# retinal-information-processing-lab/gaussian_processes

Measured on AMD Instinct MI355X. Metric: GP fits/sec (kernel+chol+solve+grad loglik) at N=8192 d=256, higher is better.
Workload: dtype f64; 1 GPU; N=8192 d=256 single cell f64, one M-step closure evaluation with 6 gradients (BASELINE configs[2], headline); N=8192, d=256, parallelism=independent units over 1 GPU(s), one process per GPU, no data-path collective

## Files before the change

gaussian_processes_amd/_lib.py:

```python
from __future__ import annotations

import ctypes
import os

from .build import lib_path

vp, i32, i64, f64 = ctypes.c_void_p, ctypes.c_int, ctypes.c_int64, ctypes.c_double
pd = ctypes.POINTER(ctypes.c_double)

_SIGS = {
    "gpfit_version": (i32, []),
    "gpfit_last_error": (ctypes.c_char_p, []),
    "gpfit_dgemm": (i32, [vp, i32, i32, i32, i32, i32, f64, vp, i64, vp, i64, f64, vp, i64, i32, i32, i32]),
    "gpfit_dgemm_ex": (i32, [vp, i32, i32, i32, i32, i32, f64, vp, i64, vp, i64, f64, vp, i64, i32, i32, i32, i32, i32]),
    "gpfit_ctx_create": (i32, [i32, i64, i64, i64, ctypes.POINTER(vp)]),
    "gpfit_ctx_destroy": (None, [vp]),
    "gpfit_check_limits": (i32, [pd, pd, pd]),
    "gpfit_localker_mask": (i32, [pd, i32, i32, vp, ctypes.POINTER(i64)]),
    "gpfit_localker": (i32, [vp, vp, pd, i32, i32, vp, i64, vp, vp]),
    "gpfit_acosker": (i32, [vp, vp, f64, vp, i64, i64, vp, i64, i64, i64, vp, i64, vp, vp, i64, vp]),
    "gpfit_acosker_pullback": (i32, [vp, vp, f64, vp, i64, i64, vp, i64, i64, i64, vp, i64, vp, i64, vp, vp, i64, pd]),
    "gpfit_acosker_diag": (i32, [vp, vp, f64, vp, i64, i64, i64, vp, i64, vp, vp, vp]),
    "gpfit_fit_eval": (i32, [vp, vp, pd, pd, pd, i32, i32, vp, i64, i64, vp, vp, vp, i64, f64, f64, i32, pd,
                             vp, vp, vp]),
    "gpfit_potrf": (i32, [vp, vp, vp, i64, i64, vp, i64, vp, i64, pd, ctypes.POINTER(i32)]),
    "gpfit_potrf_append": (i32, [vp, vp, vp, i64, vp, i64, i64, vp, pd, ctypes.POINTER(i32)]),
    "gpfit_estep": (i32, [vp, vp, vp, i64, i64, vp, vp, vp, f64, vp, vp, i64]),
    "gpfit_estep_projected": (i32, [vp, vp, vp, i64, vp, i64, vp, i64, i64, i64, vp, vp, vp, f64, vp, vp, i64, vp, vp,
                                    vp]),
# ... 65 lines not shown
```

gaussian_processes_amd/csrc/api_core.hip:

```cpp
#include "common.h"
#include "gpfit_mi355x.h"

namespace gpfit {
static thread_local std::string g_err;
void set_error(const std::string& m) { g_err = m; }
}

extern "C" {

int gpfit_version(void) { return GPFIT_VERSION; }

const char* gpfit_last_error(void) { return gpfit::g_err.c_str(); }

int gpfit_dgemm_ex(void* stream, int a_kmajor, int b_kmajor, int M, int N, int K, double alpha,
                   const double* A, int64_t lda, const double* B, int64_t ldb, double beta, double* C,
                   int64_t ldc, int out_lower, int a_tri, int b_tri, int walk, int tile);

int gpfit_dgemm(void* stream, int a_kmajor, int b_kmajor, int M, int N, int K, double alpha,
                const double* A, int64_t lda, const double* B, int64_t ldb, double beta, double* C,
                int64_t ldc, int out_lower, int a_tri, int b_tri) {
  return gpfit_dgemm_ex(stream, a_kmajor, b_kmajor, M, N, K, alpha, A, lda, B, ldb, beta, C, ldc, out_lower,
                        a_tri, b_tri, 0, 0);
}

int gpfit_dgemm_ex(void* stream, int a_kmajor, int b_kmajor, int M, int N, int K, double alpha,
                   const double* A, int64_t lda, const double* B, int64_t ldb, double beta, double* C,
                   int64_t ldc, int out_lower, int a_tri, int b_tri, int walk, int tile) {
  if ((M & 1) || (N & 1)) {
    gpfit::set_error("gpfit_dgemm: M and N must be even");
    return -3;
  }
  gpfit::GemmArgs g{};
  g.A = A; g.B = B; g.C = C;
  g.lda = lda; g.ldb = ldb; g.ldc = ldc;
  g.M = M; g.N = N; g.K = K;
  g.alpha = alpha; g.beta = beta;
  g.a_kmajor = a_kmajor; g.b_kmajor = b_kmajor;
  g.out_lower = out_lower; g.a_tri = a_tri; g.b_tri = b_tri;
  g.batch = 1; g.split_k = 1; g.reverse = walk & 15; g.tile = tile;
  g.half_occ = (walk >> 4) & 1;
  return gpfit::launch_gemm(g, (hipStream_t)stream);
}

}
```

gaussian_processes_amd/csrc/common.h:

```cpp
#pragma once
#include <hip/hip_runtime.h>
#include <stdint.h>
#include <stdio.h>
#include <string>

namespace gpfit {

constexpr double PI32 = 3.1415927410125732;

constexpr int TILE = 128;
constexpr int TRMV_ROWS = 128;
constexpr int KTILE = 16;

void set_error(const std::string& msg);

#define GP_HIP(expr)                                                                     \
  do {                                                                                   \
    hipError_t _e = (expr);                                                              \
    if (_e != hipSuccess) {                                                              \
      gpfit::set_error(std::string(#expr) + ": " + hipGetErrorString(_e));               \
      return -100;                                                                       \
    }                                                                                    \
  } while (0)

// ... 8 lines not shown
  R* C;
  int64_t lda, ldb, ldc;
  int M, N, K;
  double alpha, beta;
  int a_kmajor, b_kmajor;
  int out_lower;
  int a_tri, b_tri;
  int batch;
  int64_t sA, sB, sC;
  int split_k;
  int tile;
  int reverse;
  int workspace;
  void* sk_ws;
  int tile_limit;
  int half_occ;
  const int* sched;
  int sched_blocks;
  int epi;
  R* aux;
  double* sumsq;
  int nptr;
  const R* Ap[GEMM_MAXB];
  const R* Bp[GEMM_MAXB];
  R* Cp[GEMM_MAXB];
  R* auxp[GEMM_MAXB];
  double* sumsqp[GEMM_MAXB];
};
using GemmArgs = GemmArgsT<double>;

constexpr size_t SK_WS_BYTES = (size_t)2 * 512 * TILE * TILE * sizeof(double);

template <typename R> constexpr int ktile_of() { return 128 / (int)sizeof(R); }

template <typename R> int launch_gemm(const GemmArgsT<R>& a, hipStream_t s);
template <typename R> int gemm_pick_tile(const GemmArgsT<R>& a);
template <typename R> int launch_gemm_streamk(const GemmArgsT<R>& a, hipStream_t s);
template <typename R> int launch_gemm_plain(const GemmArgsT<R>& a, hipStream_t s);
template <typename R> bool gemm_pair_ok(const GemmArgsT<R>& a, const GemmArgsT<R>& b);
template <typename R> int launch_gemm_pair(const GemmArgsT<R>& a, const GemmArgsT<R>& b, hipStream_t s);
template <typename R> int launch_gemm_xcd(const GemmArgsT<R>& a, hipStream_t s);
template <typename R> bool gemm_epilogue_ok(const GemmArgsT<R>& a);
template <typename R> bool gemm_streamk_applies(const GemmArgsT<R>& a);
template <typename R> bool gemm_streamk_carries(const GemmArgsT<R>& a);
template <typename R> int gemm_sumsq_entries(const GemmArgsT<R>& a);
template <typename R> bool gemm_xcd_applies(const GemmArgsT<R>& a);

template <typename R>
// ... 20 lines not shown
```

gaussian_processes_amd/csrc/fit.hip:

```cpp
#include "context.h"
#include "gpfit_mi355x.h"

#include <algorithm>
#include <chrono>
#include <cmath>
#include <cstdlib>
#include <cstring>
#include <limits>

namespace gpfit {

static thread_local gpfit_ctx* g_prof = nullptr;
static thread_local void* g_main_sk_ws = nullptr;

static const int* walks() {
  static int w[7] = {3, 2, 1, 9, 9, 2, 2};
  static bool init = false;
  if (!init) {
    init = true;
    if (const char* e = getenv("GPFIT_WALKS")) {
      int v[7];
      if (sscanf(e, "%d,%d,%d,%d,%d,%d,%d", &v[0], &v[1], &v[2], &v[3], &v[4], &v[5], &v[6]) == 7)
        for (int i = 0; i < 7; ++i) w[i] = v[i];
    }
// ... 245 lines not shown
    bt.n = B.nb;
    for (int b = 0; b < B.nb; ++b) {
      bt.A[b] = B.A[b] + off(r0, r0); bt.L[b] = B.L[b] + off(r0, r0); bt.Li[b] = B.Li[b] + off(r0, r0);
      bt.info[b] = B.info[b];
    }
    bt.lda = bt.ldl = bt.ldi = ld;
    bt.info_base = r0;
    return launch_chol_leaf_batch(bt, s);
  }
  const int k = n / TILE;
  const int n1 = ((k + 1) / 2) * TILE, n2 = n - n1;
  const int r1 = r0 + n1;
  GP_TRY(potrf_lockstep<R>(B, r0, n1, all, s));
  GP_TRY(bgemm<R>(B, s, all, 0, 0, n2, n1, n1, 1.0, B.A, off(r1, r0), B.Li, off(r0, r0), 0.0, B.L, off(r1, r0), 0, 0, 2,
                  walks()[0], B.ws, B.sk_ws));
  hipEvent_t joined = nullptr;
  if (need && B.ctx && B.side_min > 0 && n >= B.side_min && B.ctx->side) {
    gpfit_ctx* c = B.ctx;
    auto next_event = [&]() {
      if (c->side_ev_next == (int)c->side_ev.size()) {
        hipEvent_t e = nullptr;
        (void)hipEventCreateWithFlags(&e, hipEventDisableTiming);
        c->side_ev.push_back(e);
      }
      return c->side_ev[c->side_ev_next++];
    };
    hipEvent_t fork = next_event();
    joined = next_event();
    GP_HIP(hipEventRecord(fork, s));
    GP_HIP(hipStreamWaitEvent(c->side, fork, 0));
    GP_TRY(bgemm<R>(B, c->side, need, 0, 1, n2, n1, n1, 1.0, B.L, off(r1, r0), B.Li, off(r0, r0), 0.0, B.Tmp, off(r1, r0), 0, 0,
                    1, walks()[1], 1, c->sk_ws[1]));
    GP_HIP(hipEventRecord(joined, c->side));
  }
  bool merged = false;
  if (need && !joined) {
    static const bool no_batch = getenv("GPFIT_NO_BATCH") != nullptr;
    const GemmArgsT<R> g2 = batch_args<R>(B, all, 0, 0, n2, n2, n1, -1.0, B.L, off(r1, r0), B.L, off(r1, r0), 1.0, B.A, off(r1, r1),
                                          1, 0, 0, 0);
    const GemmArgsT<R> g3 = batch_args<R>(B, need, 0, 1, n2, n1, n1, 1.0, B.L, off(r1, r0), B.Li, off(r0, r0), 0.0, B.Tmp,
                                          off(r1, r0), 0, 0, 1, walks()[1]);
    if (!no_batch && gemm_pair_ok(g2, g3)) {
      if (gemm_log_eval() >= 0 && g_eval_count == gemm_log_eval())
        fprintf(stderr, "[gpfit gemm] pair: M %d N %d K %d lower 1 nb %d + M %d N %d K %d btri 1 nb %d tile %d flops %.6e\n", g2.M, g2.N,
                g2.K, g2.nptr, g3.M, g3.N, g3.K, g3.nptr, gemm_pick_tile(g3), gemm_flops(g2) + gemm_flops(g3));
      ProfScope ps(s, g_prof ? gemm_flops(g2) + gemm_flops(g3) : 0.0, 3);
      GP_TRY(launch_gemm_pair(g2, g3, s));
      merged = true;
    }
  }
  if (!merged)
    GP_TRY(bgemm<R>(B, s, all, 0, 0, n2, n2, n1, -1.0, B.L, off(r1, r0), B.L, off(r1, r0), 1.0, B.A, off(r1, r1), 1, 0, 0, 0,
                    B.ws, B.sk_ws));
  GP_TRY(potrf_lockstep<R>(B, r1, n2, need | halves, s));
  if (need) {
    if (joined) GP_HIP(hipStreamWaitEvent(s, joined, 0));
    else if (!merged)
      GP_TRY(bgemm<R>(B, s, need, 0, 1, n2, n1, n1, 1.0, B.L, off(r1, r0), B.Li, off(r0, r0), 0.0, B.Tmp, off(r1, r0), 0, 0,
                      1, walks()[1], B.ws, B.sk_ws));
    GP_TRY(bgemm<R>(B, s, need, 0, 1, n2, n1, n2, -1.0, B.Li, off(r1, r1), B.Tmp, off(r1, r0), 0.0, B.Li, off(r1, r0), 0, 1, 0,
                    walks()[2], B.ws, B.sk_ws));
  }
  return 0;
}

template int potrf_lockstep<double>(const CholBatchT<double>&, int, int, uint32_t, hipStream_t, uint32_t);
template int potrf_lockstep<float>(const CholBatchT<float>&, int, int, uint32_t, hipStream_t, uint32_t);

// ... 289 lines not shown
  };
  c->phase_valid = false;
  phase(0, s);
  g_main_sk_ws = c->sk_ws[0];
  prof_begin(c);
  struct ProfGuard { gpfit_ctx* c; ~ProfGuard() { prof_end(c); } } prof_guard{c};
  GP_HIP(hipMemsetAsync(c->info, 0, 4 * sizeof(int), s));
  GP_HIP(hipMemcpyAsync(c->pix, c->pix_host, (size_t)d * sizeof(int), hipMemcpyHostToDevice, s));
  GP_HIP(hipMemsetAsync(RP(c->mpad), 0, (size_t)np * sizeof(R), s));
  GP_HIP(hipMemcpyAsync(RP(c->mpad), m, (size_t)n * sizeof(R), hipMemcpyDeviceToDevice, s));

  const bool reuse_V = (want_grad & 2) && c->lv_valid && c->lv_n == n && c->lv_bytes == (int)sizeof(R);
  const bool async_call = (want_grad & 4) != 0;
  const bool mixed_grad = (want_grad & 8) != 0 && sizeof(R) == 8 && (want_grad & 1);
  want_grad &= 1;
  static const int side_min_env = getenv("GPFIT_SIDE_MIN") ? atoi(getenv("GPFIT_SIDE_MIN")) : 1024;
  const int side_min = async_call ? 0 : side_min_env;
  if (!async_call) GP_TRY(ensure_side_stream(c));
  c->side_ev_next = 0;
  if (!reuse_V) {
    c->lv_valid = false; c->lv32_valid = false;
    GP_HIP(hipEventRecord(c->ev_fork, s));
    GP_HIP(hipStreamWaitEvent(c->aux, c->ev_fork, 0));
    GP_TRY(launch_pack_lower(V, ldv, n, RP(c->Vbuf), ld, np, c->aux));
    GP_HIP(hipEventRecord(c->ev_join, c->aux));
  }

  GP_TRY(launch_localker<R>(th, c->pix, d, dp, n_rows, n_cols, RP(c->Cmat), dp, nullptr, s));
  GP_TRY(launch_gather(X, ldx, n, c->pix, d, dp, np, RP(c->Xt), ld, RP(c->Xm), dp, s));
  GP_TRY(gemm<R>(s, 1, 1, dp, np, dp, 1.0, RP(c->Cmat), dp, RP(c->Xt), ld, 0.0, RP(c->XCt), ld, 0, 0, 0));
  GP_TRY(launch_qvec(RP(c->Xt), RP(c->XCt), ld, dp, n, np, s0sq, RP(c->Kvec), RP(c->q), s));
// ... 944 lines not shown
```

gaussian_processes_amd/csrc/gemm.hip:

```cpp
#include "gemm_core.h"

#include <algorithm>
#include <cstdlib>
#include <mutex>
#include <set>
#include <utility>

namespace gpfit {

template <typename R, bool A_KMAJOR, bool B_KMAJOR, bool EDGE, int T, int NS>
__device__ __forceinline__ bool gemm_tile_compute(const GemmArgsT<R>& p, int tiles_n, int ntiles, R* smem,
                                                  typename Real<R>::acc_t (&acc)[T / 32][T / 32], int& ti, int& tj,
                                                  int& row0, int& col0, R*& C) {
  constexpr int KT = Real<R>::KT;

  const int bid = (p.reverse & 1) ? (ntiles - 1 - (int)blockIdx.x) : (int)blockIdx.x;
  if (p.sched != nullptr) {
    const int e = p.sched[blockIdx.x];
    if (e < 0) return false;
    ti = e >> 16;
    tj = e & 0xffff;
  } else if (p.out_lower && (p.reverse & 2) && T == TILE) {
    const int nt = tiles_n;
    int j = (int)((2.0 * nt + 1.0 - sqrt((2.0 * nt + 1.0) * (2.0 * nt + 1.0) - 8.0 * (double)bid)) * 0.5);
    while (j > 0 && (long)j * nt - (long)j * (j - 1) / 2 > bid) --j;
    while ((long)(j + 1) * nt - (long)(j + 1) * j / 2 <= bid) ++j;
    tj = j;
    ti = j + (bid - (j * nt - j * (j - 1) / 2));
  } else if (p.out_lower) {
    lower_tile(bid, TILE / T, ti, tj);
  } else if (p.reverse & 2) {
    const int tiles_m = ntiles / tiles_n;
    tj = bid / tiles_m;
// ... 30 lines not shown
    kbeg = kbeg + s0 * KT;
    C += (int64_t)z * p.sC;
  }

#pragma unroll
  for (int i = 0; i < T / 32; ++i)
#pragma unroll
    for (int j = 0; j < T / 32; ++j) acc[i][j] = acc_zero<R>();

  gemm_mainloop<R, A_KMAJOR, B_KMAJOR, EDGE, T, 0, NS>(A, p.lda, B, p.ldb, p.M, p.N, row0, col0, kbeg, kend, smem, acc,
                                                       (p.reverse & 4) != 0);
  return true;
}

template <typename R, bool A_KMAJOR, bool B_KMAJOR, bool EDGE, int T, int NS, int EPI = 0>
__device__ __forceinline__ void gemm_tile_body(const GemmArgsT<R>& p, int tiles_n, int ntiles, R* smem) {
  typename Real<R>::acc_t acc[T / 32][T / 32];
  int ti, tj, row0, col0;
  R* C;
  if (!gemm_tile_compute<R, A_KMAJOR, B_KMAJOR, EDGE, T, NS>(p, tiles_n, ntiles, smem, acc, ti, tj, row0, col0, C)) return;

  const R alpha = (R)p.alpha, beta = (p.split_k > 1) ? (R)0 : (R)p.beta;
  const int64_t ldc = p.ldc;
  const int M = p.M, N = p.N;
  if constexpr (EPI != 0) {
    constexpr int epi = EPI;
    R* __restrict__ D = p.nptr > 0 ? p.auxp[blockIdx.y] : p.aux;
    double* __restrict__ sumsq = p.nptr > 0 ? p.sumsqp[blockIdx.y] : p.sumsq;
    double ss = 0.0;
    for_each_acc<R, T>(acc, row0, col0, [&](int row, int col, R v) {
      if (EDGE && !(row < M && col < N)) return;
      R o = alpha * v;
      R* c = C + (int64_t)row * ldc + col;
      if (epi & 4) {
        R* dd = D + (int64_t)row * ldc + col;
// ... 29 lines not shown
  } else {
    for_each_acc<R, T>(acc, row0, col0, [&](int row, int col, R v) {
      if (!EDGE || (row < M && col < N)) {
        R* c = C + (int64_t)row * ldc + col;
        *c = alpha * v + beta * (*c);
      }
    });
  }
}

template <typename R, bool A_KMAJOR, bool B_KMAJOR, bool EDGE, int T, int NS = 2>
__global__ __launch_bounds__(GEMM_THREADS, (T == 128 || NS > 2 ? 2 : 4)) void gemm_mfma_kernel(GemmArgsT<R> p,
                                                                                               int tiles_n,
                                                                                               int ntiles) {
  __shared__ __attribute__((aligned(16))) R smem[2 * NS * Real<R>::KT * T];
  gemm_tile_body<R, A_KMAJOR, B_KMAJOR, EDGE, T, NS>(p, tiles_n, ntiles, smem);
}

#ifdef GPFIT_CLOCK_STAMPS
__device__ long long g_gemm_clock[2][4096][2];
#endif

template <typename R, bool A_KMAJOR, bool B_KMAJOR>
__global__ __launch_bounds__(GEMM_THREADS, 2) void gemm_xcd_kernel(GemmArgsT<R> p, int tiles_n, int ntiles) {
  __shared__ __attribute__((aligned(16))) R smem[4 * Real<R>::KT * TILE];
#ifdef GPFIT_CLOCK_STAMPS
  const long long t0 = __builtin_amdgcn_s_memtime(), w0 = __builtin_amdgcn_s_memrealtime();
#endif
  gemm_tile_body<R, A_KMAJOR, B_KMAJOR, false, TILE, 2>(p, tiles_n, ntiles, smem);
#ifdef GPFIT_CLOCK_STAMPS
  if (threadIdx.x == 0 && blockIdx.x < 4096) {
    g_gemm_clock[B_KMAJOR ? 1 : 0][blockIdx.x][0] = (long long)__builtin_amdgcn_s_memtime() - t0;
    g_gemm_clock[B_KMAJOR ? 1 : 0][blockIdx.x][1] = (long long)__builtin_amdgcn_s_memrealtime() - w0;
  }
#endif
}

template <typename R, bool A_KMAJOR, bool B_KMAJOR, int EPI>
__global__ __launch_bounds__(GEMM_THREADS, 2) void gemm_epi_kernel(GemmArgsT<R> p, int tiles_n, int ntiles) {
  __shared__ __attribute__((aligned(16))) R smem[4 * Real<R>::KT * TILE];
#ifdef GPFIT_CLOCK_STAMPS
  const long long t0 = __builtin_amdgcn_s_memtime(), w0 = __builtin_amdgcn_s_memrealtime();
#endif
  gemm_tile_body<R, A_KMAJOR, B_KMAJOR, false, TILE, 2, EPI>(p, tiles_n, ntiles, smem);
#ifdef GPFIT_CLOCK_STAMPS
  if (threadIdx.x == 0 && blockIdx.x < 4096 && EPI != 4) {
    g_gemm_clock[B_KMAJOR ? 1 : 0][blockIdx.x][0] = (long long)__builtin_amdgcn_s_memtime() - t0;
    g_gemm_clock[B_KMAJOR ? 1 : 0][blockIdx.x][1] = (long long)__builtin_amdgcn_s_memrealtime() - w0;
  }
#endif
}

template <typename R>
int gemm_pick_tile(const GemmArgsT<R>& a) {
  if (a.tile == 128 || a.tile == 64 || a.tile == 32) return a.tile;
  auto ntiles = [&](int T) {
    const long tm = (a.M + T - 1) / T, tn = (a.N + T - 1) / T;
    const long nb = (a.M + TILE - 1) / TILE;
    return (a.out_lower ? (long)lower_tile_count((int)nb, TILE / T) : tm * tn) * (a.nptr > 0 ? a.nptr : (a.batch > 0 ? a.batch : 1)) *
           (a.split_k > 1 ? a.split_k : 1);
  };
  static const long t128_min = getenv("GPFIT_T128_MIN") ? atol(getenv("GPFIT_T128_MIN")) : 384;
  static const long t128_tri_min = getenv("GPFIT_T128_TRI_MIN") ? atol(getenv("GPFIT_T128_TRI_MIN")) : 1024;
  const bool batch_tri = a.nptr > 0 && (a.a_tri || a.b_tri);
  if (ntiles(128) >= (batch_tri ? t128_tri_min : t128_min)) return 128;
  static const long t64_min = getenv("GPFIT_T64_MIN") ? atol(getenv("GPFIT_T64_MIN")) : 256;
  static const long t32_dim = getenv("GPFIT_T32_DIM") ? atol(getenv("GPFIT_T32_DIM")) : 1024;
  if (ntiles(64) >= t64_min) return 64;
  return (a.M <= t32_dim && a.N <= t32_dim) ? 32 : 64;
}

constexpr int HALF_OCC_LDS = 17 * 1024;
static void allow_dynamic_lds(const void* fn) {
  static std::mutex mu;
  static std::set<std::pair<const void*, int>> done;
  int device = 0;
  (void)hipGetDevice(&device);
  std::lock_guard<std::mutex> lock(mu);
  if (done.insert({fn, device}).second)
    (void)hipFuncSetAttribute(fn, hipFuncAttributeMaxDynamicSharedMemorySize, HALF_OCC_LDS);
}

template <typename R, int T>
static void launch_T(const GemmArgsT<R>& p, hipStream_t s) {
  const int tm = (p.M + T - 1) / T, tn = (p.N + T - 1) / T;
  const int tiles = p.out_lower ? lower_tile_count((p.M + TILE - 1) / TILE, TILE / T) : tm * tn;
  const bool edge = (p.M % T) || (p.N % T) || (p.out_lower && (p.M % TILE));
  dim3 grid(p.sched ? p.sched_blocks : (p.tile_limit > 0 ? std::min(p.tile_limit, tiles) : tiles), p.batch,
            p.split_k > 1 ? p.split_k : 1);
  dim3 block(GEMM_THREADS);
  constexpr int DEEP = (T == 128) ? 2 : (T == 64 ? 4 : 8);
  static const int deep_max = getenv("GPFIT_DEEP_MAX") ? atoi(getenv("GPFIT_DEEP_MAX")) : 512;
  const bool deep = DEEP > 2 && !edge && (long)grid.x * grid.y * grid.z <= deep_max;
  const bool half = (T == TILE) && p.half_occ && !deep;
#define GP_LAUNCH(AK, BK, ED)                                                                          \
  do {                                                                                                 \
    if (deep) hipLaunchKernelGGL((gemm_mfma_kernel<R, AK, BK, ED, T, (ED ? 2 : DEEP)>), grid, block, 0, s, p, tn, tiles); \
    else if (half) {                                                                                   \
      allow_dynamic_lds(reinterpret_cast<const void*>(gemm_mfma_kernel<R, AK, BK, ED, T, 2>));          \
      hipLaunchKernelGGL((gemm_mfma_kernel<R, AK, BK, ED, T, 2>), grid, block, HALF_OCC_LDS, s, p, tn, tiles); \
    } else hipLaunchKernelGGL((gemm_mfma_kernel<R, AK, BK, ED, T, 2>), grid, block, 0, s, p, tn, tiles); \
  } while (0)
  if (p.epi) {
    if constexpr (T == TILE) {
      const int key = p.epi * 4 + (p.a_kmajor ? 2 : 0) + (p.b_kmajor ? 1 : 0);
      if (key == 2 * 4 + 1) hipLaunchKernelGGL((gemm_epi_kernel<R, false, true, 2>), grid, block, 0, s, p, tn, tiles);
      else if (key == 1 * 4 + 0) hipLaunchKernelGGL((gemm_epi_kernel<R, false, false, 1>), grid, block, 0, s, p, tn, tiles);
      else if (key == 4 * 4 + 1) hipLaunchKernelGGL((gemm_epi_kernel<R, false, true, 4>), grid, block, 0, s, p, tn, tiles);
    }
    return;
  }
  if (p.sched && T == TILE && !edge) {
    switch ((p.a_kmajor ? 2 : 0) | (p.b_kmajor ? 1 : 0)) {
      case 0: hipLaunchKernelGGL((gemm_xcd_kernel<R, false, false>), grid, block, 0, s, p, tn, tiles); break;
      case 1: hipLaunchKernelGGL((gemm_xcd_kernel<R, false, true>), grid, block, 0, s, p, tn, tiles); break;
      case 2: hipLaunchKernelGGL((gemm_xcd_kernel<R, true, false>), grid, block, 0, s, p, tn, tiles); break;
      default: hipLaunchKernelGGL((gemm_xcd_kernel<R, true, true>), grid, block, 0, s, p, tn, tiles); break;
    }
    return;
  }
  const int sel = (p.a_kmajor ? 4 : 0) | (p.b_kmajor ? 2 : 0) | (edge ? 1 : 0);
  switch (sel) {
    case 0: GP_LAUNCH(false, false, false); break;
    case 1: GP_LAUNCH(false, false, true); break;
    case 2: GP_LAUNCH(false, true, false); break;
// ... 2 lines not shown
    case 5: GP_LAUNCH(true, false, true); break;
    case 6: GP_LAUNCH(true, true, false); break;
    case 7: GP_LAUNCH(true, true, true); break;
  }
#undef GP_LAUNCH
}

template <typename R>
bool gemm_epilogue_ok(const GemmArgsT<R>& a) {
  if (a.split_k > 1 || (a.batch > 1 && a.nptr <= 0) || a.M <= 0 || a.N <= 0) return false;
  const int T = gemm_pick_tile(a);
  if ((a.M % T) || (a.N % T)) return false;
  if ((a.epi & 1) && (!a.out_lower || a.M != a.N)) return false;
  if ((a.epi & 2) && (T != TILE || !a.out_lower)) return false;
  if ((a.epi & 4) && a.nptr <= 0 && a.aux == nullptr) return false;
  if (T != TILE || a.a_kmajor || a.half_occ) return false;
  if (!((a.epi == 2 && a.b_kmajor) || (a.epi == 1 && !a.b_kmajor) || (a.epi == 4 && a.b_kmajor))) return false;
  if (a.nptr > 0) return true;
  if (T == TILE && a.tile_limit == 0) {
    if ((a.reverse & 8) && gemm_xcd_applies(a)) return true;
    if (gemm_streamk_applies(a)) return gemm_streamk_carries(a);
  }
  return true;
}

template <typename R>
int gemm_sumsq_entries(const GemmArgsT<R>& a) {
  if (!(a.epi & 2) || !gemm_epilogue_ok(a)) return 0;
  const int t = a.M / TILE, nt = t * (t + 1) / 2;
  if (a.nptr > 0 || a.half_occ || a.tile_limit != 0 || a.batch > 1) return nt;
  if ((a.reverse & 8) && gemm_xcd_applies(a)) return nt;
  return gemm_streamk_applies(a) ? 33 * nt : nt;
}
template int gemm_sumsq_entries<double>(const GemmArgsT<double>&);
template int gemm_sumsq_entries<float>(const GemmArgsT<float>&);
template bool gemm_epilogue_ok<double>(const GemmArgsT<double>&);
template bool gemm_epilogue_ok<float>(const GemmArgsT<float>&);

template <typename R>
int launch_gemm(const GemmArgsT<R>& a, hipStream_t s) {
  if (a.M <= 0 || a.N <= 0) return 0;
  if (a.epi && !gemm_epilogue_ok(a)) {
    set_error("launch_gemm: this launch cannot carry a fused epilogue (ask gemm_epilogue_ok first)");
    return -3;
  }
  if (a.nptr > 0) return launch_gemm_plain(a, s);
  if (a.half_occ) return launch_gemm_plain(a, s);
  if (a.tile_limit == 0 && gemm_pick_tile(a) == TILE && a.batch <= 1) {
    if (a.reverse & 8) {
      const int rc = launch_gemm_xcd(a, s);
      if (rc <= 0) return rc;
    }
    const int rc = launch_gemm_streamk(a, s);
    if (rc <= 0) return rc;
  }
  return launch_gemm_plain(a, s);
}

template <typename R>
int launch_gemm_plain(const GemmArgsT<R>& a, hipStream_t s) {
  if (a.M <= 0 || a.N <= 0) return 0;
  constexpr int EPC = 16 / (int)sizeof(R);
// ... 23 lines not shown
  return 0;
}

template <typename R>
struct GemmPairT {
  GemmArgsT<R> g[2];
  int tiles[2], tiles_n[2];
};

template <typename R, int T, int NS>
__global__ __launch_bounds__(GEMM_THREADS, (NS > 2 ? 2 : 4)) void gemm_pair_kernel(GemmPairT<R> q) {
  __shared__ __attribute__((aligned(16))) R smem[2 * NS * Real<R>::KT * T];
  const int w = blockIdx.z;
  const GemmArgsT<R>& p = q.g[w];
  if ((int)blockIdx.x >= q.tiles[w] || (int)blockIdx.y >= p.batch) return;
  if (p.b_kmajor) gemm_tile_body<R, false, true, false, T, NS>(p, q.tiles_n[w], q.tiles[w], smem);
  else gemm_tile_body<R, false, false, false, T, NS>(p, q.tiles_n[w], q.tiles[w], smem);
}

template <typename R>
static int pair_member_tile(const GemmArgsT<R>& a) {
  constexpr int EPC = 16 / (int)sizeof(R);
  if (a.nptr <= 0 || a.nptr > GEMM_MAXB || a.epi || a.split_k > 1 || a.sched || a.half_occ || a.tile_limit || a.a_kmajor) return 0;
  if (a.M <= 0 || a.N <= 0 || (a.M % 64) || (a.N % 64) || (a.out_lower && ((a.M % TILE) || a.M != a.N))) return 0;
  if (a.K % ktile_of<R>() != 0 || (a.lda % EPC) || (a.ldb % EPC)) return 0;
  const int T = gemm_pick_tile(a);
  return (T == 32 || T == 64) ? T : 0;
}

template <typename R>
bool gemm_pair_ok(const GemmArgsT<R>& a, const GemmArgsT<R>& b) {
  static const bool off = getenv("GPFIT_NO_PAIR") != nullptr;
  static const bool no64 = getenv("GPFIT_NO_PAIR64") != nullptr;
  if (off) return false;
  const int ta = pair_member_tile(a), tb = pair_member_tile(b);
  return ta != 0 && ta == tb && !(no64 && ta == 64);
}
template bool gemm_pair_ok<double>(const GemmArgsT<double>&, const GemmArgsT<double>&);
// ... 51 lines not shown
```

gaussian_processes_amd/csrc/gemm_streamk.hip:

```cpp
#include "gemm_core.h"

#include <algorithm>
#include <cstdlib>
#include <map>
#include <mutex>
#include <tuple>
#include <vector>

namespace gpfit {

struct SkTile {
  int row0, col0, kbeg, ksteps;
  int prefix;
};

struct SkPlan {
  SkTile* tiles = nullptr;
  int ntiles = 0;
  int total = 0;
  int blocks = 0;
  int per_block = 0;
  int* fix_tile = nullptr;
  int* fix_ptr = nullptr;
  int* fix_slot = nullptr;
// ... 16 lines not shown
  int nt_all;
};

constexpr int SK_SLOTS = 512;

template <typename R, bool A_KMAJOR, bool B_KMAJOR>
__device__ __forceinline__ void sk_segment(const SkParams<R>& p, const SkTile& tl, int kb, int ke, R* smem,
                                           typename Real<R>::acc_t (&acc)[4][4]) {
#pragma unroll
  for (int i = 0; i < 4; ++i)
#pragma unroll
    for (int j = 0; j < 4; ++j) acc[i][j] = acc_zero<R>();
  gemm_mainloop<R, A_KMAJOR, B_KMAJOR, false, TILE>(p.A, p.lda, p.B, p.ldb, p.M, p.N, tl.row0, tl.col0, kb, ke, smem, acc);
}

template <typename R, bool A_KMAJOR, bool B_KMAJOR, int EPI = 0>
__global__ __launch_bounds__(GEMM_THREADS, 2) void gemm_streamk_kernel(SkParams<R> p) {
  constexpr int KT = Real<R>::KT;
  __shared__ __attribute__((aligned(16))) R smem[4 * KT * TILE];
  int it = (int)blockIdx.x * p.per_block;
  const int it_end = min(p.total, it + p.per_block);
  if (it >= it_end) return;
  int lo = 0, hi = p.ntiles - 1;
  while (lo < hi) {
    const int mid = (lo + hi + 1) >> 1;
    if (p.tiles[mid].prefix <= it) lo = mid; else hi = mid - 1;
  }
  int t = lo, nseg = 0;
  while (it < it_end) {
    const SkTile tl = p.tiles[t];
    const int tbeg = tl.prefix, tend = tbeg + tl.ksteps;
    const int s1 = min(it_end, tend);
    const int kb = tl.kbeg + (it - tbeg) * KT, ke = tl.kbeg + (s1 - tbeg) * KT;
    typename Real<R>::acc_t acc[4][4];
    sk_segment<R, A_KMAJOR, B_KMAJOR>(p, tl, kb, ke, smem, acc);
// ... 30 lines not shown
    if (whole_done) {
    } else if (it == tbeg && s1 == tend) {
      R* __restrict__ C = p.C;
      const int64_t ldc = p.ldc;
      const R alpha = (R)p.alpha, beta = (R)p.beta;
      if (beta == (R)0) {
        for_each_acc<R, TILE>(acc, tl.row0, tl.col0,
                              [&](int row, int col, R v) { C[(int64_t)row * ldc + col] = alpha * v; });
      } else {
        for_each_acc<R, TILE>(acc, tl.row0, tl.col0, [&](int row, int col, R v) {
          R* c = C + (int64_t)row * ldc + col;
          *c = alpha * v + beta * (*c);
        });
      }
    } else {
      R* __restrict__ P = p.partial + ((int64_t)2 * blockIdx.x + (nseg > 0 ? 1 : 0)) * (TILE * TILE);
      for_each_acc<R, TILE>(acc, 0, 0, [&](int row, int col, R v) { P[row * TILE + col] = v; });
    }
    ++nseg;
    it = s1;
    ++t;
  }
}

template <typename R, int EPI = 0>
__global__ __launch_bounds__(256) void streamk_fixup_kernel(SkParams<R> p, const int* __restrict__ fix_tile,
                                                            const int* __restrict__ fix_ptr,
                                                            const int* __restrict__ fix_slot) {
  using V = typename Real<R>::vec_t;
  constexpr int EPC = Real<R>::EPC;
  const SkTile tl = p.tiles[fix_tile[blockIdx.x]];
  const int s0 = fix_ptr[blockIdx.x], s1 = fix_ptr[blockIdx.x + 1];
  const R alpha = (R)p.alpha, beta = (R)p.beta;
  const int band = TILE / (int)gridDim.y;
  double ss = 0.0;
  for (int e = threadIdx.x * EPC; e < band * TILE; e += blockDim.x * EPC) {
    const int r = blockIdx.y * band + (e >> 7), c = e & 127;
// ... 171 lines not shown
  }
  if (first > 0) {
    GemmArgsT<R> head = a;
    head.tile = TILE;
    head.tile_limit = first;
    const int rc = launch_gemm_plain(head, s);
    if (rc != 0) return rc;
  }
  SkParams<R> p{};
  p.A = a.A; p.B = a.B; p.C = a.C; p.lda = a.lda; p.ldb = a.ldb; p.ldc = a.ldc; p.M = a.M; p.N = a.N;
  p.alpha = a.alpha; p.beta = a.beta; p.tiles = plan.tiles; p.ntiles = plan.ntiles; p.total = plan.total;
  p.per_block = plan.per_block; p.partial = (R*)(a.sk_ws ? a.sk_ws : fallback_ws);
  p.sumsq = a.sumsq; p.nt_all = (a.M / TILE) * (a.M / TILE + 1) / 2;
  dim3 grid(plan.blocks), block(GEMM_THREADS);
  const int sel = (a.a_kmajor ? 2 : 0) | (a.b_kmajor ? 1 : 0);
  if (a.epi == 0) switch (sel) {
    case 0: hipLaunchKernelGGL((gemm_streamk_kernel<R, false, false>), grid, block, 0, s, p); break;
    case 1: hipLaunchKernelGGL((gemm_streamk_kernel<R, false, true>), grid, block, 0, s, p); break;
    case 2: hipLaunchKernelGGL((gemm_streamk_kernel<R, true, false>), grid, block, 0, s, p); break;
    case 3: hipLaunchKernelGGL((gemm_streamk_kernel<R, true, true>), grid, block, 0, s, p); break;
  }
  if (a.epi == 0) {
    if (plan.nfix)
      hipLaunchKernelGGL(streamk_fixup_kernel<R>, dim3(plan.nfix, 32), dim3(256), 0, s, p, plan.fix_tile, plan.fix_ptr,
                         plan.fix_slot);
    GP_HIP(hipGetLastError());
    return 0;
  }
  if (a.epi == 2) {
    hipLaunchKernelGGL((gemm_streamk_kernel<R, false, true, 2>), grid, block, 0, s, p);
    if (plan.nfix)
// ... 13 lines not shown
```

include/gpfit_mi355x.h:

```cpp
#ifndef GPFIT_MI355X_H
#define GPFIT_MI355X_H

#include <stdint.h>

#ifdef __cplusplus
extern "C" {
#endif

#define GPFIT_VERSION 100

int gpfit_version(void);
const char* gpfit_last_error(void);

int gpfit_dgemm(void* stream, int a_kmajor, int b_kmajor, int M, int N, int K, double alpha,
                const double* A, int64_t lda, const double* B, int64_t ldb, double beta, double* C,
                int64_t ldc, int out_lower, int a_tri, int b_tri);
int gpfit_dgemm_ex(void* stream, int a_kmajor, int b_kmajor, int M, int N, int K, double alpha,
                   const double* A, int64_t lda, const double* B, int64_t ldb, double beta, double* C,
                   int64_t ldc, int out_lower, int a_tri, int b_tri, int walk, int tile);

typedef struct gpfit_ctx gpfit_ctx;
int gpfit_ctx_create(int device, int64_t n_max, int64_t d_max, int64_t d_full_max, gpfit_ctx** out);
void gpfit_ctx_destroy(gpfit_ctx* ctx);

int gpfit_check_limits(const double* theta, const double* lower, const double* upper);

int gpfit_localker_mask(const double* theta, int n_rows, int n_cols, uint8_t* mask_host, int64_t* d_out);

int gpfit_localker(gpfit_ctx* ctx, void* stream, const double* theta, int n_rows, int n_cols,
                   const uint8_t* mask_host, int64_t d, double* C, double* dC);

int gpfit_acosker(gpfit_ctx* ctx, void* stream, double sigma0, const double* x1, int64_t ld1, int64_t n1,
                  const double* x2, int64_t ld2, int64_t n2, int64_t d, const double* C, int64_t ldC,
// ... 93 lines not shown
```

Baseline: 34.23 fits/s.

## Run side-stream Cholesky GEMM as a persistent background kernel on reserved CUs

Replaces the half-occupancy GEMM mode with a persistent 'background' GEMM kernel. It runs a grid of fewer CUs than the device has (reserving 16 by default), loops over virtual blocks, and uses extra dynamic LDS. The side-stream L*Linv product in the blocked Cholesky now uses this kernel, and the main-stream trailing update is issued before the fork, so the two can overlap without the side kernel taking every CU. The side-stream threshold is raised from 1024 to 4096, and an sgemm_ex entry point is added. The risks are a slower side product on fewer CUs and a changed ordering of work on the main stream.

New measurement: 34.30 fits/s (median of 6 runs). About the same (+0.2%).

```diff
diff --git a/gaussian_processes_amd/_lib.py b/gaussian_processes_amd/_lib.py
--- a/gaussian_processes_amd/_lib.py
+++ b/gaussian_processes_amd/_lib.py
@@ -13,6 +13,7 @@
     "gpfit_last_error": (ctypes.c_char_p, []),
     "gpfit_dgemm": (i32, [vp, i32, i32, i32, i32, i32, f64, vp, i64, vp, i64, f64, vp, i64, i32, i32, i32]),
     "gpfit_dgemm_ex": (i32, [vp, i32, i32, i32, i32, i32, f64, vp, i64, vp, i64, f64, vp, i64, i32, i32, i32, i32, i32]),
+    "gpfit_sgemm_ex": (i32, [vp, i32, i32, i32, i32, i32, f64, vp, i64, vp, i64, f64, vp, i64, i32, i32, i32, i32, i32]),
     "gpfit_ctx_create": (i32, [i32, i64, i64, i64, ctypes.POINTER(vp)]),
     "gpfit_ctx_destroy": (None, [vp]),
     "gpfit_check_limits": (i32, [pd, pd, pd]),
diff --git a/gaussian_processes_amd/csrc/api_core.hip b/gaussian_processes_amd/csrc/api_core.hip
--- a/gaussian_processes_amd/csrc/api_core.hip
+++ b/gaussian_processes_amd/csrc/api_core.hip
@@ -1,9 +1,37 @@
 #include "common.h"
 #include "gpfit_mi355x.h"
+
+#include <algorithm>
+#include <cstdlib>
 
 namespace gpfit {
 static thread_local std::string g_err;
 void set_error(const std::string& m) { g_err = m; }
+
+int gemm_bg_reserve_default() {
+  static const int v = getenv("GPFIT_BG_RESERVE") ? atoi(getenv("GPFIT_BG_RESERVE")) : 16;
+  return v;
+}
+
+template <typename R>
+static int gemm_ex(void* stream, int a_kmajor, int b_kmajor, int M, int N, int K, double alpha, const R* A, int64_t lda,
+                   const R* B, int64_t ldb, double beta, R* C, int64_t ldc, int out_lower, int a_tri, int b_tri, int walk,
+                   int tile) {
+  if ((M & 1) || (N & 1)) {
+    set_error("gpfit_dgemm: M and N must be even");
+    return -3;
+  }
+  GemmArgsT<R> g{};
+  g.A = A; g.B = B; g.C = C;
+  g.lda = lda; g.ldb = ldb; g.ldc = ldc;
+  g.M = M; g.N = N; g.K = K;
+  g.alpha = alpha; g.beta = beta;
+  g.a_kmajor = a_kmajor; g.b_kmajor = b_kmajor;
+  g.out_lower = out_lower; g.a_tri = a_tri; g.b_tri = b_tri;
+  g.batch = 1; g.split_k = 1; g.reverse = walk & 15; g.tile = tile;
+  if (walk & 32) g.background = ((walk >> 8) & 255) ? ((walk >> 8) & 255) : std::max(1, gemm_bg_reserve_default());
+  return launch_gemm(g, (hipStream_t)stream);
+}
 }
 
 extern "C" {
@@ -26,20 +54,15 @@
 int gpfit_dgemm_ex(void* stream, int a_kmajor, int b_kmajor, int M, int N, int K, double alpha,
                    const double* A, int64_t lda, const double* B, int64_t ldb, double beta, double* C,
                    int64_t ldc, int out_lower, int a_tri, int b_tri, int walk, int tile) {
-  if ((M & 1) || (N & 1)) {
-    gpfit::set_error("gpfit_dgemm: M and N must be even");
-    return -3;
-  }
-  gpfit::GemmArgs g{};
-  g.A = A; g.B = B; g.C = C;
-  g.lda = lda; g.ldb = ldb; g.ldc = ldc;
-  g.M = M; g.N = N; g.K = K;
-  g.alpha = alpha; g.beta = beta;
-  g.a_kmajor = a_kmajor; g.b_kmajor = b_kmajor;
-  g.out_lower = out_lower; g.a_tri = a_tri; g.b_tri = b_tri;
-  g.batch = 1; g.split_k = 1; g.reverse = walk & 15; g.tile = tile;
-  g.half_occ = (walk >> 4) & 1;
-  return gpfit::launch_gemm(g, (hipStream_t)stream);
+  return gpfit::gemm_ex<double>(stream, a_kmajor, b_kmajor, M, N, K, alpha, A, lda, B, ldb, beta, C, ldc, out_lower, a_tri,
+                                b_tri, walk, tile);
+}
+
+int gpfit_sgemm_ex(void* stream, int a_kmajor, int b_kmajor, int M, int N, int K, double alpha,
+                   const float* A, int64_t lda, const float* B, int64_t ldb, double beta, float* C,
+                   int64_t ldc, int out_lower, int a_tri, int b_tri, int walk, int tile) {
+  return gpfit::gemm_ex<float>(stream, a_kmajor, b_kmajor, M, N, K, alpha, A, lda, B, ldb, beta, C, ldc, out_lower, a_tri,
+                               b_tri, walk, tile);
 }
 
 }
diff --git a/gaussian_processes_amd/csrc/common.h b/gaussian_processes_amd/csrc/common.h
--- a/gaussian_processes_amd/csrc/common.h
+++ b/gaussian_processes_amd/csrc/common.h
@@ -46,7 +46,7 @@
   int workspace;
   void* sk_ws;
   int tile_limit;
-  int half_occ;
+  int background;
   const int* sched;
   int sched_blocks;
   int epi;
@@ -64,6 +64,11 @@
 constexpr size_t SK_WS_BYTES = (size_t)2 * 512 * TILE * TILE * sizeof(double);
 
 template <typename R> constexpr int ktile_of() { return 128 / (int)sizeof(R); }
+
+constexpr int GEMM_BG_LDS = 17 * 1024;
+void gemm_bg_allow_lds(const void* fn);
+int gemm_bg_grid(int reserve);
+int gemm_bg_reserve_default();
 
 template <typename R> int launch_gemm(const GemmArgsT<R>& a, hipStream_t s);
 template <typename R> int gemm_pick_tile(const GemmArgsT<R>& a);
diff --git a/gaussian_processes_amd/csrc/fit.hip b/gaussian_processes_amd/csrc/fit.hip
--- a/gaussian_processes_amd/csrc/fit.hip
+++ b/gaussian_processes_amd/csrc/fit.hip
@@ -283,8 +283,28 @@
   GP_TRY(potrf_lockstep<R>(B, r0, n1, all, s));
   GP_TRY(bgemm<R>(B, s, all, 0, 0, n2, n1, n1, 1.0, B.A, off(r1, r0), B.Li, off(r0, r0), 0.0, B.L, off(r1, r0), 0, 0, 2,
                   walks()[0], B.ws, B.sk_ws));
+  const bool side = need && B.ctx && B.side_min > 0 && n >= B.side_min && B.ctx->side;
+  bool merged = false;
+  if (need && !side) {
+    static const bool no_batch = getenv("GPFIT_NO_BATCH") != nullptr;
+    const GemmArgsT<R> g2 = batch_args<R>(B, all, 0, 0, n2, n2, n1, -1.0, B.L, off(r1, r0), B.L, off(r1, r0), 1.0, B.A, off(r1, r1),
+                                          1, 0, 0, 0);
+    const GemmArgsT<R> g3 = batch_args<R>(B, need, 0, 1, n2, n1, n1, 1.0, B.L, off(r1, r0), B.Li, off(r0, r0), 0.0, B.Tmp,
+                                          off(r1, r0), 0, 0, 1, walks()[1]);
+    if (!no_batch && gemm_pair_ok(g2, g3)) {
+      if (gemm_log_eval() >= 0 && g_eval_count == gemm_log_eval())
+        fprintf(stderr, "[gpfit gemm] pair: M %d N %d K %d lower 1 nb %d + M %d N %d K %d btri 1 nb %d tile %d flops %.6e\n", g2.M, g2.N,
+                g2.K, g2.nptr, g3.M, g3.N, g3.K, g3.nptr, gemm_pick_tile(g3), gemm_flops(g2) + gemm_flops(g3));
+      ProfScope ps(s, g_prof ? gemm_flops(g2) + gemm_flops(g3) : 0.0, 3);
+      GP_TRY(launch_gemm_pair(g2, g3, s));
+      merged = true;
+    }
+  }
+  if (!merged)
+    GP_TRY(bgemm<R>(B, s, all, 0, 0, n2, n2, n1, -1.0, B.L, off(r1, r0), B.L, off(r1, r0), 1.0, B.A, off(r1, r1), 1, 0, 0, 0,
+                    B.ws, B.sk_ws));
   hipEvent_t joined = nullptr;
-  if (need && B.ctx && B.side_min > 0 && n >= B.side_min && B.ctx->side) {
+  if (side) {
     gpfit_ctx* c = B.ctx;
     auto next_event = [&]() {
       if (c->side_ev_next == (int)c->side_ev.size()) {
@@ -297,30 +317,24 @@
     hipEvent_t fork = next_event();
     joined = next_event();
     GP_HIP(hipEventRecord(fork, s));
-    GP_HIP(hipStreamWaitEvent(c->side, fork, 0));
-    GP_TRY(bgemm<R>(B, c->side, need, 0, 1, n2, n1, n1, 1.0, B.L, off(r1, r0), B.Li, off(r0, r0), 0.0, B.Tmp, off(r1, r0), 0, 0,
-                    1, walks()[1], 1, c->sk_ws[1]));
+    static const bool host_fork = getenv("GPFIT_SIDE_FORK") && !strcmp(getenv("GPFIT_SIDE_FORK"), "host");
+    static const bool side_bg = !(getenv("GPFIT_SIDE_BG") && atoi(getenv("GPFIT_SIDE_BG")) == 0);
+    if (host_fork) GP_HIP(hipEventSynchronize(fork));
+    else GP_HIP(hipStreamWaitEvent(c->side, fork, 0));
+    if (side_bg) {
+      for (int b = 0; b < B.nb; ++b)
+        if (need & (1u << b)) {
+          GemmArgsT<R> g = gemm_args<R>(0, 1, n2, n1, n1, 1.0, B.L[b] + off(r1, r0), ld, B.Li[b] + off(r0, r0), ld, 0.0,
+                                        B.Tmp[b] + off(r1, r0), ld, 0, 0, 1, walks()[1], 1, c->sk_ws[1]);
+          g.background = std::max(1, gemm_bg_reserve_default());
+          GP_TRY(run_gemm(c->side, g));
+        }
+    } else {
+      GP_TRY(bgemm<R>(B, c->side, need, 0, 1, n2, n1, n1, 1.0, B.L, off(r1, r0), B.Li, off(r0, r0), 0.0, B.Tmp, off(r1, r0), 0, 0,
+                      1, walks()[1], 1, c->sk_ws[1]));
+    }
     GP_HIP(hipEventRecord(joined, c->side));
   }
-  bool merged = false;
-  if (need && !joined) {
-    static const bool no_batch = getenv("GPFIT_NO_BATCH") != nullptr;
-    const GemmArgsT<R> g2 = batch_args<R>(B, all, 0, 0, n2, n2, n1, -1.0, B.L, off(r1, r0), B.L, off(r1, r0), 1.0, B.A, off(r1, r1),
-                                          1, 0, 0, 0);
-    const GemmArgsT<R> g3 = batch_args<R>(B, need, 0, 1, n2, n1, n1, 1.0, B.L, off(r1, r0), B.Li, off(r0, r0), 0.0, B.Tmp,
-                                          off(r1, r0), 0, 0, 1, walks()[1]);
-    if (!no_batch && gemm_pair_ok(g2, g3)) {
-      if (gemm_log_eval() >= 0 && g_eval_count == gemm_log_eval())
-        fprintf(stderr, "[gpfit gemm] pair: M %d N %d K %d lower 1 nb %d + M %d N %d K %d btri 1 nb %d tile %d flops %.6e\n", g2.M, g2.N,
-                g2.K, g2.nptr, g3.M, g3.N, g3.K, g3.nptr, gemm_pick_tile(g3), gemm_flops(g2) + gemm_flops(g3));
-      ProfScope ps(s, g_prof ? gemm_flops(g2) + gemm_flops(g3) : 0.0, 3);
-      GP_TRY(launch_gemm_pair(g2, g3, s));
-      merged = true;
-    }
-  }
-  if (!merged)
-    GP_TRY(bgemm<R>(B, s, all, 0, 0, n2, n2, n1, -1.0, B.L, off(r1, r0), B.L, off(r1, r0), 1.0, B.A, off(r1, r1), 1, 0, 0, 0,
-                    B.ws, B.sk_ws));
   GP_TRY(potrf_lockstep<R>(B, r1, n2, need | halves, s));
   if (need) {
     if (joined) GP_HIP(hipStreamWaitEvent(s, joined, 0));
@@ -640,7 +654,7 @@
   const bool async_call = (want_grad & 4) != 0;
   const bool mixed_grad = (want_grad & 8) != 0 && sizeof(R) == 8 && (want_grad & 1);
   want_grad &= 1;
-  static const int side_min_env = getenv("GPFIT_SIDE_MIN") ? atoi(getenv("GPFIT_SIDE_MIN")) : 1024;
+  static const int side_min_env = getenv("GPFIT_SIDE_MIN") ? atoi(getenv("GPFIT_SIDE_MIN")) : 4096;
   const int side_min = async_call ? 0 : side_min_env;
   if (!async_call) GP_TRY(ensure_side_stream(c));
   c->side_ev_next = 0;
diff --git a/gaussian_processes_amd/csrc/gemm.hip b/gaussian_processes_amd/csrc/gemm.hip
--- a/gaussian_processes_amd/csrc/gemm.hip
+++ b/gaussian_processes_amd/csrc/gemm.hip
@@ -2,6 +2,7 @@
 
 #include <algorithm>
 #include <cstdlib>
+#include <map>
 #include <mutex>
 #include <set>
 #include <utility>
@@ -11,12 +12,12 @@
 template <typename R, bool A_KMAJOR, bool B_KMAJOR, bool EDGE, int T, int NS>
 __device__ __forceinline__ bool gemm_tile_compute(const GemmArgsT<R>& p, int tiles_n, int ntiles, R* smem,
                                                   typename Real<R>::acc_t (&acc)[T / 32][T / 32], int& ti, int& tj,
-                                                  int& row0, int& col0, R*& C) {
+                                                  int& row0, int& col0, R*& C, int vb) {
   constexpr int KT = Real<R>::KT;
 
-  const int bid = (p.reverse & 1) ? (ntiles - 1 - (int)blockIdx.x) : (int)blockIdx.x;
+  const int bid = (p.reverse & 1) ? (ntiles - 1 - vb) : vb;
   if (p.sched != nullptr) {
-    const int e = p.sched[blockIdx.x];
+    const int e = p.sched[vb];
     if (e < 0) return false;
     ti = e >> 16;
     tj = e & 0xffff;
@@ -77,11 +78,11 @@
 }
 
 template <typename R, bool A_KMAJOR, bool B_KMAJOR, bool EDGE, int T, int NS, int EPI = 0>
-__device__ __forceinline__ void gemm_tile_body(const GemmArgsT<R>& p, int tiles_n, int ntiles, R* smem) {
+__device__ __forceinline__ void gemm_tile_body(const GemmArgsT<R>& p, int tiles_n, int ntiles, R* smem, int vb) {
   typename Real<R>::acc_t acc[T / 32][T / 32];
   int ti, tj, row0, col0;
   R* C;
-  if (!gemm_tile_compute<R, A_KMAJOR, B_KMAJOR, EDGE, T, NS>(p, tiles_n, ntiles, smem, acc, ti, tj, row0, col0, C)) return;
+  if (!gemm_tile_compute<R, A_KMAJOR, B_KMAJOR, EDGE, T, NS>(p, tiles_n, ntiles, smem, acc, ti, tj, row0, col0, C, vb)) return;
 
   const R alpha = (R)p.alpha, beta = (p.split_k > 1) ? (R)0 : (R)p.beta;
   const int64_t ldc = p.ldc;
@@ -141,7 +142,7 @@
                                                                                                int tiles_n,
                                                                                                int ntiles) {
   __shared__ __attribute__((aligned(16))) R smem[2 * NS * Real<R>::KT * T];
-  gemm_tile_body<R, A_KMAJOR, B_KMAJOR, EDGE, T, NS>(p, tiles_n, ntiles, smem);
+  gemm_tile_body<R, A_KMAJOR, B_KMAJOR, EDGE, T, NS>(p, tiles_n, ntiles, smem, (int)blockIdx.x);
 }
 
 #ifdef GPFIT_CLOCK_STAMPS
@@ -154,7 +155,7 @@
 #ifdef GPFIT_CLOCK_STAMPS
   const long long t0 = __builtin_amdgcn_s_memtime(), w0 = __builtin_amdgcn_s_memrealtime();
 #endif
-  gemm_tile_body<R, A_KMAJOR, B_KMAJOR, false, TILE, 2>(p, tiles_n, ntiles, smem);
+  gemm_tile_body<R, A_KMAJOR, B_KMAJOR, false, TILE, 2>(p, tiles_n, ntiles, smem, (int)blockIdx.x);
 #ifdef GPFIT_CLOCK_STAMPS
   if (threadIdx.x == 0 && blockIdx.x < 4096) {
     g_gemm_clock[B_KMAJOR ? 1 : 0][blockIdx.x][0] = (long long)__builtin_amdgcn_s_memtime() - t0;
@@ -169,13 +170,20 @@
 #ifdef GPFIT_CLOCK_STAMPS
   const long long t0 = __builtin_amdgcn_s_memtime(), w0 = __builtin_amdgcn_s_memrealtime();
 #endif
-  gemm_tile_body<R, A_KMAJOR, B_KMAJOR, false, TILE, 2, EPI>(p, tiles_n, ntiles, smem);
+  gemm_tile_body<R, A_KMAJOR, B_KMAJOR, false, TILE, 2, EPI>(p, tiles_n, ntiles, smem, (int)blockIdx.x);
 #ifdef GPFIT_CLOCK_STAMPS
   if (threadIdx.x == 0 && blockIdx.x < 4096 && EPI != 4) {
     g_gemm_clock[B_KMAJOR ? 1 : 0][blockIdx.x][0] = (long long)__builtin_amdgcn_s_memtime() - t0;
     g_gemm_clock[B_KMAJOR ? 1 : 0][blockIdx.x][1] = (long long)__builtin_amdgcn_s_memrealtime() - w0;
   }
 #endif
+}
+
+template <typename R, bool A_KMAJOR, bool B_KMAJOR>
+__global__ __launch_bounds__(GEMM_THREADS, 2) void gemm_bg_kernel(GemmArgsT<R> p, int tiles_n, int ntiles, int nvb) {
+  __shared__ __attribute__((aligned(16))) R smem[4 * Real<R>::KT * TILE];
+  for (int vb = (int)blockIdx.x; vb < nvb; vb += (int)gridDim.x)
+    gemm_tile_body<R, A_KMAJOR, B_KMAJOR, false, TILE, 2>(p, tiles_n, ntiles, smem, vb);
 }
 
 template <typename R>
@@ -197,15 +205,32 @@
   return (a.M <= t32_dim && a.N <= t32_dim) ? 32 : 64;
 }
 
-constexpr int HALF_OCC_LDS = 17 * 1024;
-static void allow_dynamic_lds(const void* fn) {
+void gemm_bg_allow_lds(const void* fn) {
   static std::mutex mu;
   static std::set<std::pair<const void*, int>> done;
   int device = 0;
   (void)hipGetDevice(&device);
   std::lock_guard<std::mutex> lock(mu);
   if (done.insert({fn, device}).second)
-    (void)hipFuncSetAttribute(fn, hipFuncAttributeMaxDynamicSharedMemorySize, HALF_OCC_LDS);
+    (void)hipFuncSetAttribute(fn, hipFuncAttributeMaxDynamicSharedMemorySize, GEMM_BG_LDS);
+}
+
+int gemm_bg_grid(int reserve) {
+  static std::mutex mu;
+  static std::map<int, int> cus;
+  int device = 0;
+  (void)hipGetDevice(&device);
+  int n;
+  {
+    std::lock_guard<std::mutex> lock(mu);
+    auto it = cus.find(device);
+    if (it == cus.end()) {
+      hipDeviceProp_t prop;
+      it = cus.emplace(device, hipGetDeviceProperties(&prop, device) == hipSuccess ? prop.multiProcessorCount : 256).first;
+    }
+    n = it->second;
+  }
+  return std::max(8, 8 * ((n - std::max(0, reserve)) / 8));
 }
 
 template <typename R, int T>
@@ -219,14 +244,10 @@
   constexpr int DEEP = (T == 128) ? 2 : (T == 64 ? 4 : 8);
   static const int deep_max = getenv("GPFIT_DEEP_MAX") ? atoi(getenv("GPFIT_DEEP_MAX")) : 512;
   const bool deep = DEEP > 2 && !edge && (long)grid.x * grid.y * grid.z <= deep_max;
-  const bool half = (T == TILE) && p.half_occ && !deep;
 #define GP_LAUNCH(AK, BK, ED)                                                                          \
   do {                                                                                                 \
     if (deep) hipLaunchKernelGGL((gemm_mfma_kernel<R, AK, BK, ED, T, (ED ? 2 : DEEP)>), grid, block, 0, s, p, tn, tiles); \
-    else if (half) {                                                                                   \
-      allow_dynamic_lds(reinterpret_cast<const void*>(gemm_mfma_kernel<R, AK, BK, ED, T, 2>));          \
-      hipLaunchKernelGGL((gemm_mfma_kernel<R, AK, BK, ED, T, 2>), grid, block, HALF_OCC_LDS, s, p, tn, tiles); \
-    } else hipLaunchKernelGGL((gemm_mfma_kernel<R, AK, BK, ED, T, 2>), grid, block, 0, s, p, tn, tiles); \
+    else hipLaunchKernelGGL((gemm_mfma_kernel<R, AK, BK, ED, T, 2>), grid, block, 0, s, p, tn, tiles); \
   } while (0)
   if (p.epi) {
     if constexpr (T == TILE) {
@@ -236,6 +257,25 @@
       else if (key == 4 * 4 + 1) hipLaunchKernelGGL((gemm_epi_kernel<R, false, true, 4>), grid, block, 0, s, p, tn, tiles);
     }
     return;
+  }
+  if constexpr (T == TILE) {
+    if (p.background > 0) {
+      const int nvb = (int)grid.x;
+      const dim3 bg(std::min(nvb, gemm_bg_grid(p.background)));
+#define GP_BG(AK, BK)                                                                           \
+  do {                                                                                          \
+    gemm_bg_allow_lds(reinterpret_cast<const void*>(gemm_bg_kernel<R, AK, BK>));                  \
+    hipLaunchKernelGGL((gemm_bg_kernel<R, AK, BK>), bg, block, GEMM_BG_LDS, s, p, tn, tiles, nvb); \
+  } while (0)
+      switch ((p.a_kmajor ? 2 : 0) | (p.b_kmajor ? 1 : 0)) {
+        case 0: GP_BG(false, false); break;
+        case 1: GP_BG(false, true); break;
+        case 2: GP_BG(true, false); break;
+        default: GP_BG(true, true); break;
+      }
+#undef GP_BG
+      return;
+    }
   }
   if (p.sched && T == TILE && !edge) {
     switch ((p.a_kmajor ? 2 : 0) | (p.b_kmajor ? 1 : 0)) {
@@ -268,7 +308,7 @@
   if ((a.epi & 1) && (!a.out_lower || a.M != a.N)) return false;
   if ((a.epi & 2) && (T != TILE || !a.out_lower)) return false;
   if ((a.epi & 4) && a.nptr <= 0 && a.aux == nullptr) return false;
-  if (T != TILE || a.a_kmajor || a.half_occ) return false;
+  if (T != TILE || a.a_kmajor || a.background) return false;
   if (!((a.epi == 2 && a.b_kmajor) || (a.epi == 1 && !a.b_kmajor) || (a.epi == 4 && a.b_kmajor))) return false;
   if (a.nptr > 0) return true;
   if (T == TILE && a.tile_limit == 0) {
@@ -282,7 +322,7 @@
 int gemm_sumsq_entries(const GemmArgsT<R>& a) {
   if (!(a.epi & 2) || !gemm_epilogue_ok(a)) return 0;
   const int t = a.M / TILE, nt = t * (t + 1) / 2;
-  if (a.nptr > 0 || a.half_occ || a.tile_limit != 0 || a.batch > 1) return nt;
+  if (a.nptr > 0 || a.tile_limit != 0 || a.batch > 1) return nt;
   if ((a.reverse & 8) && gemm_xcd_applies(a)) return nt;
   return gemm_streamk_applies(a) ? 33 * nt : nt;
 }
@@ -298,8 +338,16 @@
     set_error("launch_gemm: this launch cannot carry a fused epilogue (ask gemm_epilogue_ok first)");
     return -3;
   }
+  if (a.background > 0 && a.tile != TILE) {
+    GemmArgsT<R> b = a;
+    b.tile = TILE;
+    return launch_gemm(b, s);
+  }
+  if (a.background > 0 && (a.epi || a.nptr > 0 || a.batch > 1 || a.split_k > 1 || (a.M % TILE) || (a.N % TILE))) {
+    set_error("launch_gemm: a background launch is one plain product on full 128-tiles");
+    return -3;
+  }
   if (a.nptr > 0) return launch_gemm_plain(a, s);
-  if (a.half_occ) return launch_gemm_plain(a, s);
   if (a.tile_limit == 0 && gemm_pick_tile(a) == TILE && a.batch <= 1) {
     if (a.reverse & 8) {
       const int rc = launch_gemm_xcd(a, s);
@@ -353,14 +401,14 @@
   const int w = blockIdx.z;
   const GemmArgsT<R>& p = q.g[w];
   if ((int)blockIdx.x >= q.tiles[w] || (int)blockIdx.y >= p.batch) return;
-  if (p.b_kmajor) gemm_tile_body<R, false, true, false, T, NS>(p, q.tiles_n[w], q.tiles[w], smem);
-  else gemm_tile_body<R, false, false, false, T, NS>(p, q.tiles_n[w], q.tiles[w], smem);
+  if (p.b_kmajor) gemm_tile_body<R, false, true, false, T, NS>(p, q.tiles_n[w], q.tiles[w], smem, (int)blockIdx.x);
+  else gemm_tile_body<R, false, false, false, T, NS>(p, q.tiles_n[w], q.tiles[w], smem, (int)blockIdx.x);
 }
 
 template <typename R>
 static int pair_member_tile(const GemmArgsT<R>& a) {
   constexpr int EPC = 16 / (int)sizeof(R);
-  if (a.nptr <= 0 || a.nptr > GEMM_MAXB || a.epi || a.split_k > 1 || a.sched || a.half_occ || a.tile_limit || a.a_kmajor) return 0;
+  if (a.nptr <= 0 || a.nptr > GEMM_MAXB || a.epi || a.split_k > 1 || a.sched || a.background || a.tile_limit || a.a_kmajor) return 0;
   if (a.M <= 0 || a.N <= 0 || (a.M % 64) || (a.N % 64) || (a.out_lower && ((a.M % TILE) || a.M != a.N))) return 0;
   if (a.K % ktile_of<R>() != 0 || (a.lda % EPC) || (a.ldb % EPC)) return 0;
   const int T = gemm_pick_tile(a);
diff --git a/gaussian_processes_amd/csrc/gemm_streamk.hip b/gaussian_processes_amd/csrc/gemm_streamk.hip
--- a/gaussian_processes_amd/csrc/gemm_streamk.hip
+++ b/gaussian_processes_amd/csrc/gemm_streamk.hip
@@ -54,11 +54,10 @@
   gemm_mainloop<R, A_KMAJOR, B_KMAJOR, false, TILE>(p.A, p.lda, p.B, p.ldb, p.M, p.N, tl.row0, tl.col0, kb, ke, smem, acc);
 }
 
-template <typename R, bool A_KMAJOR, bool B_KMAJOR, int EPI = 0>
-__global__ __launch_bounds__(GEMM_THREADS, 2) void gemm_streamk_kernel(SkParams<R> p) {
+template <typename R, bool A_KMAJOR, bool B_KMAJOR, int EPI>
+__device__ __forceinline__ void sk_share(const SkParams<R>& p, int vb, R* smem) {
   constexpr int KT = Real<R>::KT;
-  __shared__ __attribute__((aligned(16))) R smem[4 * KT * TILE];
-  int it = (int)blockIdx.x * p.per_block;
+  int it = vb * p.per_block;
   const int it_end = min(p.total, it + p.per_block);
   if (it >= it_end) return;
   int lo = 0, hi = p.ntiles - 1;
@@ -119,13 +118,25 @@
         });
       }
     } else {
-      R* __restrict__ P = p.partial + ((int64_t)2 * blockIdx.x + (nseg > 0 ? 1 : 0)) * (TILE * TILE);
+      R* __restrict__ P = p.partial + ((int64_t)2 * vb + (nseg > 0 ? 1 : 0)) * (TILE * TILE);
       for_each_acc<R, TILE>(acc, 0, 0, [&](int row, int col, R v) { P[row * TILE + col] = v; });
     }
     ++nseg;
     it = s1;
     ++t;
   }
+}
+
+template <typename R, bool A_KMAJOR, bool B_KMAJOR, int EPI = 0>
+__global__ __launch_bounds__(GEMM_THREADS, 2) void gemm_streamk_kernel(SkParams<R> p) {
+  __shared__ __attribute__((aligned(16))) R smem[4 * Real<R>::KT * TILE];
+  sk_share<R, A_KMAJOR, B_KMAJOR, EPI>(p, (int)blockIdx.x, smem);
+}
+
+template <typename R, bool A_KMAJOR, bool B_KMAJOR>
+__global__ __launch_bounds__(GEMM_THREADS, 2) void gemm_streamk_bg_kernel(SkParams<R> p, int nvb) {
+  __shared__ __attribute__((aligned(16))) R smem[4 * Real<R>::KT * TILE];
+  for (int vb = (int)blockIdx.x; vb < nvb; vb += (int)gridDim.x) sk_share<R, A_KMAJOR, B_KMAJOR, 0>(p, vb, smem);
 }
 
 template <typename R, int EPI = 0>
@@ -327,7 +338,21 @@
   p.sumsq = a.sumsq; p.nt_all = (a.M / TILE) * (a.M / TILE + 1) / 2;
   dim3 grid(plan.blocks), block(GEMM_THREADS);
   const int sel = (a.a_kmajor ? 2 : 0) | (a.b_kmajor ? 1 : 0);
-  if (a.epi == 0) switch (sel) {
+  if (a.background > 0 && a.epi == 0) {
+    const dim3 bg(std::min(plan.blocks, gemm_bg_grid(a.background)));
+#define GP_BG(AK, BK)                                                                               \
+  do {                                                                                              \
+    gemm_bg_allow_lds(reinterpret_cast<const void*>(gemm_streamk_bg_kernel<R, AK, BK>));              \
+    hipLaunchKernelGGL((gemm_streamk_bg_kernel<R, AK, BK>), bg, block, GEMM_BG_LDS, s, p, plan.blocks); \
+  } while (0)
+    switch (sel) {
+      case 0: GP_BG(false, false); break;
+      case 1: GP_BG(false, true); break;
+      case 2: GP_BG(true, false); break;
+      case 3: GP_BG(true, true); break;
+    }
+#undef GP_BG
+  } else if (a.epi == 0) switch (sel) {
     case 0: hipLaunchKernelGGL((gemm_streamk_kernel<R, false, false>), grid, block, 0, s, p); break;
     case 1: hipLaunchKernelGGL((gemm_streamk_kernel<R, false, true>), grid, block, 0, s, p); break;
     case 2: hipLaunchKernelGGL((gemm_streamk_kernel<R, true, false>), grid, block, 0, s, p); break;
diff --git a/include/gpfit_mi355x.h b/include/gpfit_mi355x.h
--- a/include/gpfit_mi355x.h
+++ b/include/gpfit_mi355x.h
@@ -17,6 +17,9 @@
                 int64_t ldc, int out_lower, int a_tri, int b_tri);
 int gpfit_dgemm_ex(void* stream, int a_kmajor, int b_kmajor, int M, int N, int K, double alpha,
                    const double* A, int64_t lda, const double* B, int64_t ldb, double beta, double* C,
+                   int64_t ldc, int out_lower, int a_tri, int b_tri, int walk, int tile);
+int gpfit_sgemm_ex(void* stream, int a_kmajor, int b_kmajor, int M, int N, int K, double alpha,
+                   const float* A, int64_t lda, const float* B, int64_t ldb, double beta, float* C,
                    int64_t ldc, int out_lower, int a_tri, int b_tri, int walk, int tile);
 
 typedef struct gpfit_ctx gpfit_ctx;
```
